# YzM1a0/MuDPT

Measured on AMD Instinct MI355X. Metric: images/sec fwd+bwd ViT-B/16 MuDPT, higher is better.
Workload: dtype bf16; 1 GPU; MuDPT ViT-B/16 fwd+bwd+SGD, batch 256/GPU, 11 class prompts, n_ctx 4, depth 12, synthetic 224x224 N(0,1) images, random-init frozen CLIP (BASELINE configs[1]); global_batch=256, parallelism=dp1

## Files before the change

mudpt_amd/csrc/gemm.hip:

```cpp
#include <type_traits>

#include "kernels.h"

namespace mudpt {

using gptr_t = const __attribute__((address_space(1))) void*;
using lptr_t = __attribute__((address_space(3))) void*;

template <typename T, int BM, int BN, int WM, int WN, int EPI, int NS = 2, int BK = 64>
__global__ __launch_bounds__(WM* WN * 64) void gemm_nt_kernel(GemmArgs p) {
    using elem = typename T::elem;
    using vec8 = typename T::vec8;
    constexpr int NW = WM * WN;
    static_assert(BK == 64 || BK == 128, "K-tile");
    constexpr int ROWB = BK * 2;
    constexpr int RPI = 1024 / ROWB;
    constexpr int CPR = ROWB / 16;
    constexpr int TM = BM / WM / 16;
    constexpr int TN = BN / WN / 16;
    constexpr int IA = BM / RPI / NW;
    constexpr int IB = BN / RPI / NW;
    constexpr int STAGE_BYTES = (BM + BN) * ROWB;
    static_assert(BM % (RPI * NW) == 0 && BN % (RPI * NW) == 0, "tile rows must split over the waves");

// ... 302 lines not shown
    ARG_CHECK(!a.gelu_q8 || ((epi == EPI_GELU && !a.out1_lo) || epi == EPI_GELU_BWD), "gemm: gelu_q8 belongs to the QuickGELU epilogues (1 without a split output, 3)");
    ARG_CHECK(a.lo_mode == LO_NONE || a.lo_mode == LO_F16 || a.lo_mode == LO_F8, "gemm: bad lo_mode %d", a.lo_mode);
    if (a.lo_mode != LO_NONE) ARG_CHECK(a.A_lo && (uintptr_t)a.A_lo % 16 == 0, "gemm: a split operand needs its low half (16-byte aligned)");
    if (a.lo_mode == LO_F8) {
        ARG_CHECK(dtype == DT_F16, "gemm: the e4m3 second pass exists for fp16 operands only");
        ARG_CHECK(a.B8 && (uintptr_t)a.B8 % 16 == 0 && a.K % 128 == 0, "gemm: the e4m3 second pass needs B8 and K %% 128 == 0 (K = %d)", a.K);
        ARG_CHECK(a.b8_scale > 0 && a.b8_scale < 255, "gemm: bad E8M0 weight scale %d", a.b8_scale);
    }
    if (epi == EPI_RESIDUAL || epi == EPI_GELU_BWD) ARG_CHECK(a.aux && a.ldaux >= a.N && a.ldaux % 4 == 0, "gemm: epilogue needs aux");
    if (epi == EPI_PATCH) ARG_CHECK(a.pos && a.patches > 0 && a.seq_len > a.patches && a.M % a.patches == 0, "gemm: bad patch epilogue args");
    GemmArgs b = a;
    if (variant & 0x100) b.flags |= 1;
    if (variant & 0x200) b.flags |= 2;
    b.flags |= ((variant >> 10) & 3) << 4;
    b.flags |= ((variant >> 12) & 0xff) << 8;
    if (gemm_uses_pp(epi, a, o.variant)) return launch_gemm_pp(dtype, epi, b, s, o);
    bool deep = false;
    if (const int S = split_k_slices(epi, a, o, deep); S > 1) {
        GemmArgs q = b;
        q.bias = nullptr; q.out0 = o.scratch; q.ldo0 = a.N; q.ksplit = a.K / S; q.split_stride = (size_t)a.M * a.N;
        if (dtype == DT_BF16) { if (int rc = deep ? launch_cfg<BF16, 64, 64, 2, 2, EPI_STORE_F32, 2, 128>(q, s) : launch_cfg<BF16, 64, 64, 2, 2, EPI_STORE_F32, 2>(q, s)) return rc; }
        else if (dtype == DT_F16) { if (int rc = deep ? launch_cfg<F16, 64, 64, 2, 2, EPI_STORE_F32, 2, 128>(q, s) : launch_cfg<F16, 64, 64, 2, 2, EPI_STORE_F32, 2>(q, s)) return rc; }
        else { set_error("gemm: unknown dtype %d", dtype); return MUDPT_ERR_ARG; }
        const unsigned grid = (unsigned)(((size_t)a.M * (a.N / 4) + 255) / 256);
        if (epi == EPI_STORE_F32) hipLaunchKernelGGL((splitk_reduce_kernel<BF16, true>), dim3(grid), dim3(256), 0, s, o.scratch, S, q.split_stride, a.M, a.N, a.bias, a.out0, a.ldo0);
        else if (dtype == DT_BF16) hipLaunchKernelGGL((splitk_reduce_kernel<BF16, false>), dim3(grid), dim3(256), 0, s, o.scratch, S, q.split_stride, a.M, a.N, a.bias, a.out0, a.ldo0);
        else hipLaunchKernelGGL((splitk_reduce_kernel<F16, false>), dim3(grid), dim3(256), 0, s, o.scratch, S, q.split_stride, a.M, a.N, a.bias, a.out0, a.ldo0);
        HIP_TRY(hipGetLastError());
        return MUDPT_OK;
    }
    if (dtype == DT_BF16) return launch_t<BF16>(epi, b, s, o.variant);
// ... 7 lines not shown
```

mudpt_amd/csrc/kernels.h:

```cpp
#pragma once
#include "common.h"

namespace mudpt {

enum Epilogue : int {
    EPI_STORE = 0,
    EPI_GELU = 1,
    EPI_RESIDUAL = 2,
    EPI_GELU_BWD = 3,
    EPI_PATCH = 4,
    EPI_STORE_F32 = 5
};

struct GemmArgs {
    const void* A = nullptr;
    const void* B = nullptr;
    int M = 0, N = 0, K = 0, lda = 0, ldb = 0;
    const float* bias = nullptr;
    void* out0 = nullptr; int ldo0 = 0;
    void* out1 = nullptr; int ldo1 = 0;
    void* out1_lo = nullptr;
    int out1_lo_mode = LO_F16;
    const void* A_lo = nullptr; int lo_mode = LO_NONE;
    const void* B8 = nullptr; int b8_scale = 127;
    const void* aux = nullptr; int ldaux = 0;
    bool gelu_q8 = false;
    int flags = 0;
    int patches = 0, seq_len = 0;
    const float* pos = nullptr;
    int ksplit = 0; size_t split_stride = 0;
};
struct GemmOpts {
    int variant = 0;
    hipEvent_t ev_start = nullptr, ev_stop = nullptr;
    float* scratch = nullptr; size_t scratch_elems = 0;
};
int launch_gemm(int dtype, int epi, const GemmArgs& a, hipStream_t s, const GemmOpts& o = GemmOpts());
bool gemm_uses_pp(int epi, const GemmArgs& a, int variant = 0);
int launch_gemm_pp(int dtype, int epi, const GemmArgs& a, hipStream_t s, const GemmOpts& o);

struct LnFwdArgs {
    const float* x = nullptr; int ldx = 0;
    const int* row_index = nullptr;
    const float* gamma = nullptr; const float* beta = nullptr;
    void* out = nullptr; int ldo = 0;
    void* out_lo = nullptr;
    int lo_mode = LO_F16;
    float* mean = nullptr; float* rstd = nullptr;
    int rows = 0, d = 0; bool out_f32 = false;
    const float* add = nullptr; int ldadd = 0;
    const void* add_lp = nullptr;
    float* xout = nullptr; int ldxout = 0;
    const float* ov_rows = nullptr; int ov_row0 = 0, ov_n = 0, ov_L = 1;
};
int launch_ln_fwd(int dtype, const LnFwdArgs& a, hipStream_t s, const LaunchProf* prof = nullptr);

struct LnBwdArgs {
    const void* dy = nullptr; int lddy = 0; bool dy_f32 = false;
    const float* x = nullptr; int ldx = 0;
    const int* row_index = nullptr;
    const float* mean = nullptr; const float* rstd = nullptr; const float* gamma = nullptr;
    const float* dres = nullptr; int lddres = 0;
    const void* dres_lp = nullptr;
    float* dx = nullptr; int lddx = 0;
    void* dx_lp = nullptr; int lddx_lp = 0;
    int rows = 0, d = 0;
    bool by_token = false;
    bool stats_by_token = false;
    float* side = nullptr; int side_row0 = 0, side_n = 0, side_L = 1; size_t side_ldb = 0;
};
int launch_ln_bwd(int dtype, const LnBwdArgs& a, hipStream_t s, const LaunchProf* prof = nullptr);

struct AttnArgs {
    const void* qkv = nullptr;
    void* out = nullptr;
    void* out_lo = nullptr;
    int lo_mode = LO_F16;
    int ld_out = 0;
    float* lse = nullptr;
    const void* dout = nullptr;
    void* dqkv = nullptr;
// ... 73 lines not shown
```

mudpt_amd/csrc/layernorm.hip:

```cpp
#include "kernels.h"

namespace mudpt {

constexpr int LN_MAXV = 4;

template <typename T, bool OUT_F32>
__global__ __launch_bounds__(256) void ln_fwd_kernel(LnFwdArgs p) {
    using elem = typename T::elem;
    const int lane = threadIdx.x & 63;
    const int r = blockIdx.x * 4 + (threadIdx.x >> 6);
    if (r >= p.rows) return;
    const size_t xr = p.row_index ? (size_t)p.row_index[r] : (size_t)r;
    const f32x4* x = (const f32x4*)(p.x + xr * p.ldx);
    const int d4 = p.d >> 2;
    f32x4 v[LN_MAXV];
    float s = 0.f;
    const f32x4* ov = nullptr;
    if (p.ov_rows) {
        const int pos = r % p.ov_L - p.ov_row0;
        if (pos >= 0 && pos < p.ov_n) ov = (const f32x4*)(p.ov_rows + (size_t)pos * p.d);
    }
    const f32x4* add = (p.add && !ov) ? (const f32x4*)(p.add + xr * p.ldadd) : nullptr;
    const typename T::vec4* add_lp = (p.add_lp && !ov) ? (const typename T::vec4*)((const elem*)p.add_lp + xr * p.ldadd) : nullptr;
#pragma unroll
    for (int k = 0; k < LN_MAXV; ++k) {
// ... 42 lines not shown
                    if (p.lo_mode == LO_F8) ((uint32_t*)((char*)p.out_lo + (size_t)r * p.ldo * 2))[i] = pack_lo8(rem[0], rem[1], rem[2], rem[3]);
                    else ((typename T::vec4*)((elem*)p.out_lo + (size_t)r * p.ldo))[i] = lo;
                } else {
                    typename T::vec4 o = {(elem)y[0], (elem)y[1], (elem)y[2], (elem)y[3]};
                    ((typename T::vec4*)((elem*)p.out + (size_t)r * p.ldo))[i] = o;
                }
            }
        }
    }
}

template <typename T, bool DY_F32>
__global__ __launch_bounds__(256) void ln_bwd_kernel(LnBwdArgs p) {
    using elem = typename T::elem;
    const int lane = threadIdx.x & 63;
    const int r = blockIdx.x * 4 + (threadIdx.x >> 6);
    if (r >= p.rows) return;
    const size_t t = p.row_index ? (size_t)p.row_index[r] : (size_t)r;
    const f32x4* x = (const f32x4*)(p.x + t * p.ldx);
    const int d4 = p.d >> 2;
    const size_t sr = p.by_token ? t : (size_t)r;
    const size_t st = (p.by_token || p.stats_by_token) ? t : (size_t)r;
    const float mean = p.mean[st], rstd = p.rstd[st];
    f32x4* side_row = nullptr;
    if (p.side) {
        const int pos = (int)(t % (size_t)p.side_L) - p.side_row0;
        if (pos >= 0 && pos < p.side_n) side_row = (f32x4*)(p.side + (t / (size_t)p.side_L) * p.side_ldb + (size_t)pos * p.d);
    }
    f32x4 xh[LN_MAXV], g[LN_MAXV];
    typename T::vec4 rv[LN_MAXV];
    float s1 = 0.f, s2 = 0.f;
// ... 36 lines not shown
            }
            if (side_row) { side_row[i] = dx; dx = f32x4{0.f, 0.f, 0.f, 0.f}; }
            if (p.dx) ((f32x4*)(p.dx + t * p.lddx))[i] = dx;
            if (p.dx_lp) {
                typename T::vec4 o = {(elem)dx[0], (elem)dx[1], (elem)dx[2], (elem)dx[3]};
                ((typename T::vec4*)((elem*)p.dx_lp + t * p.lddx_lp))[i] = o;
            }
        }
    }
}

int launch_ln_fwd(int dtype, const LnFwdArgs& a, hipStream_t s, const LaunchProf* prof) {
    ARG_CHECK(a.x && a.gamma && a.beta && a.out, "ln_fwd: null operand");
    ARG_CHECK(a.rows > 0 && a.d > 0 && a.d % 4 == 0 && a.d <= 256 * LN_MAXV, "ln_fwd: bad shape rows=%d d=%d", a.rows, a.d);
    ARG_CHECK(a.ldx % 4 == 0 && a.ldo % 4 == 0 && a.ldx >= a.d && a.ldo >= a.d, "ln_fwd: bad strides %d/%d", a.ldx, a.ldo);
    const dim3 grid((a.rows + 3) / 4), block(256);
    if (dtype == DT_BF16) {
        if (a.out_f32) MUDPT_LAUNCH((ln_fwd_kernel<BF16, true>), grid, block, 0, s, prof, a);
        else MUDPT_LAUNCH((ln_fwd_kernel<BF16, false>), grid, block, 0, s, prof, a);
    } else if (dtype == DT_F16) {
        if (a.out_f32) MUDPT_LAUNCH((ln_fwd_kernel<F16, true>), grid, block, 0, s, prof, a);
        else MUDPT_LAUNCH((ln_fwd_kernel<F16, false>), grid, block, 0, s, prof, a);
    } else {
        set_error("ln_fwd: unknown dtype %d", dtype);
        return MUDPT_ERR_ARG;
    }
    HIP_TRY(hipGetLastError());
    return MUDPT_OK;
}

int launch_ln_bwd(int dtype, const LnBwdArgs& a, hipStream_t s, const LaunchProf* prof) {
    ARG_CHECK(a.dy && a.x && a.mean && a.rstd && a.gamma && (a.dx || a.dx_lp), "ln_bwd: null operand");
    ARG_CHECK(!(a.dres && a.dres_lp), "ln_bwd: dres and dres_lp are exclusive");
    ARG_CHECK(!a.side || (!a.row_index && a.side_L > 0 && a.side_n > 0), "ln_bwd: the fused splice backward needs the identity row map");
    ARG_CHECK(a.rows > 0 && a.d > 0 && a.d % 4 == 0 && a.d <= 256 * LN_MAXV, "ln_bwd: bad shape rows=%d d=%d", a.rows, a.d);
    ARG_CHECK(a.ldx % 4 == 0 && a.lddy % 4 == 0 && a.lddx % 4 == 0, "ln_bwd: strides must be multiples of 4");
    const dim3 grid((a.rows + 3) / 4), block(256);
    if (dtype == DT_BF16) {
        if (a.dy_f32) MUDPT_LAUNCH((ln_bwd_kernel<BF16, true>), grid, block, 0, s, prof, a);
        else MUDPT_LAUNCH((ln_bwd_kernel<BF16, false>), grid, block, 0, s, prof, a);
    } else if (dtype == DT_F16) {
        if (a.dy_f32) MUDPT_LAUNCH((ln_bwd_kernel<F16, true>), grid, block, 0, s, prof, a);
        else MUDPT_LAUNCH((ln_bwd_kernel<F16, false>), grid, block, 0, s, prof, a);
    } else {
        set_error("ln_bwd: unknown dtype %d", dtype);
        return MUDPT_ERR_ARG;
    }
    HIP_TRY(hipGetLastError());
    return MUDPT_OK;
}

}
// ... 1 lines not shown
```

mudpt_amd/csrc/model.cpp:

```cpp
#include <dlfcn.h>
#include <stdarg.h>
#include <stdio.h>
#include <string.h>

#include <algorithm>
#include <cmath>
#include <string>
#include <vector>

#include "../../include/mudpt.h"
#include "kernels.h"

namespace mudpt {

static thread_local char g_err[1024] = "";
void set_error(const char* fmt, ...) {
    va_list ap;
    va_start(ap, fmt);
    vsnprintf(g_err, sizeof(g_err), fmt, ap);
    va_end(ap);
}
const char* get_error() { return g_err; }

static inline uint16_t f32_to_bf16(float f) {
// ... 53 lines not shown
    bool may_split = false;
    int sites = 0x1f;
    void *h_lo = nullptr, *g_lo = nullptr, *attn_lo = nullptr;
    void *h_sel_lo = nullptr, *g_sel_lo = nullptr, *attn_sel_lo = nullptr;
    int prompt_row0 = 0;
    std::vector<BlockW> w;
    std::vector<BlockAct> a;
    void *h = nullptr, *g = nullptr;
    bool exact_attn = false;
    float* qkv32 = nullptr;
    float* dx = nullptr; void* dx_lp = nullptr;
    void *dattn = nullptr, *dqkv = nullptr;
    float* delta = nullptr;
    float* upd = nullptr;
    const int* tail_rows = nullptr;
    float *xin_sel = nullptr, *xmid_sel = nullptr, *xout_sel = nullptr;
    void *attn_sel = nullptr, *h_sel = nullptr, *u_sel = nullptr, *g_sel = nullptr, *dattn_sel = nullptr;
    float* dsel = nullptr; void* dsel_lp = nullptr;
    void *q_sel = nullptr, *dq_sel = nullptr, *dqx_sel = nullptr;
    float* lse_sel = nullptr;
    const int* head_rows = nullptr;
    int head_n = 0;
    void *hd_dqkv = nullptr, *hd_h = nullptr;
    std::vector<void*> act_allocs;
    struct Seg { int row0 = 0, seq0 = 0, nseq = 0, L = 0; size_t lse0 = 0; };
    std::vector<Seg> segs;
    int rows = 0;
    const int* tail_local = nullptr;
};

// ... 63 lines not shown
    bool attn_fused_w1 = false;
    bool split_k = true;
    bool fwd_split_k = true;
    bool train_fwd = false;
    static constexpr size_t kFwdSplitTiles = 320;
    static constexpr size_t kScratchElems = (size_t)4 << 20;
    float *gemm_scratch = nullptr, *gemm_scratch2 = nullptr;
    bool attn_window = true;
    bool last_single = true;
    bool attn_two_kernels = false;
    int cocoop_chunk = 0;
    int txt_chunk = 1;
    bool any_weight_set = false;
    hipStream_t s2 = nullptr;
    hipEvent_t ev_fork = nullptr, ev_join = nullptr, ev_fork_b = nullptr, ev_join_b = nullptr;
    bool prof = false;
    int prof_mask = 0;
    int prof_stride = 1;
    long pp_seen = 0;
    std::vector<hipEvent_t> ev;
    size_t ev_used = 0;
    struct ProfRec { int cls; double work; };
    std::vector<ProfRec> ev_rec;
    double exec_flop = 0;
};
enum ProfClass : int { PC_GEMM = 0, PC_LN_FWD = 1, PC_LN_BWD = 2, PC_ATTN_FWD = 3, PC_ATTN_BWD = 4, PC_COUNT = 5 };

static int prof_next(mudpt_model* m, int cls, double work, LaunchProf* out) {
    *out = LaunchProf();
    if (!m->prof || !(m->prof_mask & (1 << cls))) return MUDPT_OK;
    if (m->ev_used + 2 > m->ev.size()) {
        for (int i = 0; i < 512; ++i) {
            hipEvent_t e;
            HIP_TRY(hipEventCreate(&e));
            m->ev.push_back(e);
        }
    }
    out->start = m->ev[m->ev_used];
    out->stop = m->ev[m->ev_used + 1];
    m->ev_used += 2;
    m->ev_rec.push_back({cls, work});
    return MUDPT_OK;
}

static int gemm_call(mudpt_model* m, int epi, const GemmArgs& a, hipStream_t s, bool bwd = false, bool fwd_split = false) {
    GemmOpts o;
    o.variant = m->gemm_variant;
    const bool fwd_small = fwd_split && m->fwd_split_k && m->train_fwd && (size_t)((a.M + 63) / 64) * ((a.N + 63) / 64) <= mudpt_model::kFwdSplitTiles;
    if (m->split_k && (bwd || fwd_small)) {
        o.scratch = s == m->s2 ? m->gemm_scratch2 : m->gemm_scratch;
        o.scratch_elems = mudpt_model::kScratchElems;
    }
    if (m->prof) m->exec_flop += 2.0 * a.M * a.N * a.K;
    if (!m->prof || !gemm_uses_pp(epi, a, o.variant)) return launch_gemm(m->dtype, epi, a, s, o);
    if (m->prof_stride > 1 && (m->pp_seen++ % m->prof_stride) != 0) return launch_gemm(m->dtype, epi, a, s, o);
    LaunchProf lp;
    if (int rc = prof_next(m, PC_GEMM, 2.0 * a.M * a.N * a.K, &lp)) return rc;
    o.ev_start = lp.start;
    o.ev_stop = lp.stop;
    return launch_gemm(m->dtype, epi, a, s, o);
}

static bool prof_big(const mudpt_model* m, const Tower& t, int rows) { return m->prof && &t == &m->vis && rows >= 4096; }
static int ln_fwd_call(mudpt_model* m, const Tower& t, const LnFwdArgs& a, hipStream_t s) {
    if (!prof_big(m, t, a.rows)) return launch_ln_fwd(m->dtype, a, s);
    const double per_elem = 4.0 + (a.add ? 4.0 : 0.0) + (a.add_lp ? 2.0 : 0.0) + (a.xout ? 4.0 : 0.0) + (a.out_f32 ? 4.0 : 2.0) + (a.out_lo ? 2.0 : 0.0);
    LaunchProf lp;
    if (int rc = prof_next(m, PC_LN_FWD, per_elem * a.rows * a.d, &lp)) return rc;
    return launch_ln_fwd(m->dtype, a, s, &lp);
}
static int ln_bwd_call(mudpt_model* m, const Tower& t, const LnBwdArgs& a, hipStream_t s) {
    if (!prof_big(m, t, a.rows)) return launch_ln_bwd(m->dtype, a, s);
    const double per_elem = (a.dy_f32 ? 4.0 : 2.0) + 4.0 + (a.dres ? 4.0 : 0.0) + (a.dres_lp ? 2.0 : 0.0) + (a.dx ? 4.0 : 0.0) + (a.dx_lp ? 2.0 : 0.0);
    LaunchProf lp;
    if (int rc = prof_next(m, PC_LN_BWD, per_elem * a.rows * a.d, &lp)) return rc;
    return launch_ln_bwd(m->dtype, a, s, &lp);
}
static int attn_call(mudpt_model* m, const Tower& t, const AttnArgs& a0, bool bwd, hipStream_t s) {
    AttnArgs a = a0;
    a.two_kernels = m->attn_two_kernels;
    a.fused_w1 = m->attn_fused_w1;
    const double prod = 2.0 * a.L * (double)a.L * 64.0 * a.H * a.B * (a.causal ? 0.5 : 1.0);
    const bool exact_fwd = !bwd && a.qkv32;
    if (m->prof && !a.sel_rows && !exact_fwd) m->exec_flop += (bwd ? 7.0 : 2.0) * prod;
    if (exact_fwd) return launch_attn_fwd_exact(a, s);
    if (!prof_big(m, t, a.B * a.L) || a.sel_rows) return bwd ? launch_attn_bwd(m->dtype, a, s) : launch_attn_fwd(m->dtype, a, s);
    const double tok = (double)a.B * a.L * a.H * 128.0;
    LaunchProf lp;
    if (int rc = prof_next(m, bwd ? PC_ATTN_BWD : PC_ATTN_FWD, bwd ? 8.0 * tok : (4.0 + (a.out_lo ? 1.0 : 0.0)) * tok, &lp)) return rc;
    return bwd ? launch_attn_bwd(m->dtype, a, s, &lp) : launch_attn_fwd(m->dtype, a, s, &lp);
}

// ... 171 lines not shown
        ALLOC(m->vis_deep, dn * dv * 4); ALLOC(m->txt_deep, dn * dt * 4);
        ALLOC(m->vsplice, (size_t)B * dn * dv * 4);
        ALLOC(m->d_vis_deep, dn * dv * 4); ALLOC(m->d_txt_deep, dn * dt * 4); ALLOC(m->d_vprompt0, (size_t)n * dv * 4);
        ALLOC(m->img_f, (size_t)B * e * 4); ALLOC(m->txt_f, (size_t)TS * e * 4); ALLOC(m->img_n, (size_t)B * e * 4); ALLOC(m->txt_n, (size_t)TS * e * 4);
        ALLOC(m->img_inv, B * 4); ALLOC(m->txt_inv, TS * 4);
        ALLOC(m->logits, (size_t)B * C * 4); ALLOC(m->dlogits, (size_t)B * C * 4); ALLOC(m->row_loss, B * 4);
        ALLOC(m->dimg, (size_t)B * e * 4); ALLOC(m->dtxt, (size_t)TS * e * 4); ALLOC(m->loss, 16);
        if (cocoop) {
            m->hid = e / 16;
            ALLOC(m->mn_hid, (size_t)B * m->hid * 4); ALLOC(m->mn_dhid, (size_t)B * m->hid * 4);
            ALLOC(m->mn_bias, (size_t)B * dt * 4); ALLOC(m->mn_dbias, (size_t)B * dt * 4);
        }
        ALLOC(m->gemm_scratch, mudpt_model::kScratchElems * 4); ALLOC(m->gemm_scratch2, mudpt_model::kScratchElems * 4);
        HIP_TRY(hipStreamCreateWithFlags(&m->s2, hipStreamNonBlocking));
        for (hipEvent_t* e : {&m->ev_fork, &m->ev_join, &m->ev_fork_b, &m->ev_join_b}) HIP_TRY(hipEventCreateWithFlags(e, hipEventDisableTiming));
        std::vector<int> cr(B), pr((size_t)B * n);
        for (int b = 0; b < B; ++b) {
            cr[b] = b * Lv;
            for (int i = 0; i < n; ++i) pr[(size_t)b * n + i] = b * Lv + (Lv - n) + i;
        }
        HIP_TRY(hipMemcpy(m->cls_rows, cr.data(), cr.size() * 4, hipMemcpyHostToDevice));
        m->vis.tail_rows = m->cls_rows;
        m->vis.head_rows = cocoop ? nullptr : m->vprompt_rows;
        ALLOC(m->tprompt_rows, (size_t)TS * n * 4);
        m->txt.head_rows = m->tprompt_rows;
        m->txt.tail_rows = m->eot_rows;
        HIP_TRY(hipMemcpy(m->vprompt_rows, pr.data(), pr.size() * 4, hipMemcpyHostToDevice));
        return MUDPT_OK;
    };
    if (int r = body()) return fail(r);
// ... 11 lines not shown
                          "visual.ln_pre.bias", "visual.ln_post.weight", "visual.ln_post.bias", "visual.proj", "positional_embedding",
                          "ln_final.weight", "ln_final.bias", "text_projection", "logit_scale"})
        m->missing.push_back(k);
    expect_block_keys(m, "visual.transformer", c->v_layers);
    expect_block_keys(m, "transformer", c->t_layers);
    *out = m;
    return MUDPT_OK;
}

extern "C" int mudpt_destroy(mudpt_model* m) {
    if (!m) return MUDPT_OK;
    for (void* p : m->allocs) (void)hipFree(p);
    for (Tower* t : {&m->vis, &m->txt})
        for (void* p : t->act_allocs) (void)hipFree(p);
    for (hipEvent_t e : m->ev) (void)hipEventDestroy(e);
    for (hipEvent_t e : {m->ev_fork, m->ev_join, m->ev_fork_b, m->ev_join_b})
        if (e) (void)hipEventDestroy(e);
    if (m->s2) (void)hipStreamDestroy(m->s2);
    delete m;
    return MUDPT_OK;
}

static int upload_f32(float* dst, const float* src, size_t n) {
    HIP_TRY(hipMemcpy(dst, src, n * 4, hipMemcpyHostToDevice));
    return MUDPT_OK;
}
static int upload_lp(int dtype, void* dst, void* dst_t, const float* src, size_t rows, size_t cols) {
    std::vector<uint16_t> tmp(rows * cols);
    auto cv = [&](float f) { return dtype == DT_BF16 ? f32_to_bf16(f) : f32_to_f16(f); };
    for (size_t i = 0; i < rows * cols; ++i) tmp[i] = cv(src[i]);
    HIP_TRY(hipMemcpy(dst, tmp.data(), tmp.size() * 2, hipMemcpyHostToDevice));
    if (dst_t) {
        for (size_t r = 0; r < rows; ++r)
// ... 293 lines not shown
    if (m_fc != LO_NONE) { l2.out_lo = t.h_sel_lo; l2.lo_mode = m_fc; }
    TRY(launch_ln_fwd(dt, l2, s));
    GemmArgs f; f.A = t.h_sel; f.lda = d; f.B = w.w_fc; f.ldb = d; f.M = S; f.N = 4 * d; f.K = d; f.bias = w.b_fc;
    split_operand(f, m_fc, t.h_sel_lo, w.w_fc8, w.s_fc8);
    f.out0 = t.u_sel; f.ldo0 = 4 * d; f.out1 = t.g_sel; f.ldo1 = 4 * d;
    f.gelu_q8 = m->gelu_q8 && t.split == LO_NONE;
    if (m_proj != LO_NONE) { f.out1_lo = t.g_sel_lo; f.out1_lo_mode = m_proj; }
    TRY(gemm_call(m, EPI_GELU, f, s));
    GemmArgs p; p.A = t.g_sel; p.lda = 4 * d; p.B = w.w_proj; p.ldb = 4 * d; p.M = S; p.N = d; p.K = 4 * d; p.bias = w.b_proj;
    split_operand(p, m_proj, t.g_sel_lo, w.w_proj8, w.s_proj8);
    p.out0 = t.xout_sel; p.ldo0 = d; p.aux = t.xmid_sel; p.ldaux = d;
    TRY(gemm_call(m, EPI_RESIDUAL, p, s));
    return MUDPT_OK;
}

static int block_fwd(mudpt_model* m, Tower& t, int i, int nseq, const float* splice, hipStream_t s) {
    const int M = tower_rows(t, nseq), d = t.d, dt = m->dtype, n = m->cfg.n_ctx;
    const std::vector<Tower::Seg> segs = tower_segs(t, nseq);
    const bool lp = m->lp_upd;
    BlockW& w = t.w[i];
    BlockAct& a = t.a[i];
    const size_t esz = 2;
    const int m_qkv = site_mode(t, SITE_QKV, d), m_out = site_mode(t, SITE_OUT, d), m_fc = site_mode(t, SITE_FC, d), m_proj = site_mode(t, SITE_PROJ, 4 * d);
    LnFwdArgs l1; l1.x = a.x_in; l1.ldx = d; l1.gamma = w.ln1_g; l1.beta = w.ln1_b; l1.out = t.h; l1.ldo = d; l1.mean = a.mean1; l1.rstd = a.rstd1; l1.rows = M; l1.d = d;
    if (m_qkv != LO_NONE) { l1.out_lo = t.h_lo; l1.lo_mode = m_qkv; }
    if (i > 0) {
        l1.x = t.a[i - 1].x_mid; l1.ldadd = d; l1.xout = a.x_in; l1.ldxout = d;
        if (lp) l1.add_lp = t.upd; else l1.add = t.upd;
        if (splice) { l1.ov_rows = splice; l1.ov_row0 = t.prompt_row0; l1.ov_n = n; l1.ov_L = t.L; }
    }
    if (splice && i > 0 && segs.size() > 1) {
        for (const Tower::Seg& g : segs) {
            LnFwdArgs b = l1;
            const size_t r0 = (size_t)g.row0;
            b.x = l1.x + r0 * l1.ldx; b.xout = l1.xout + r0 * l1.ldxout;
            if (l1.add) b.add = l1.add + r0 * l1.ldadd;
            if (l1.add_lp) b.add_lp = (const char*)l1.add_lp + r0 * l1.ldadd * esz;
            b.out = (char*)l1.out + r0 * l1.ldo * esz;
            if (l1.out_lo) b.out_lo = (char*)l1.out_lo + r0 * l1.ldo * esz;
            b.mean = l1.mean + r0; b.rstd = l1.rstd + r0; b.rows = g.nseq * g.L; b.ov_L = g.L;
            TRY(ln_fwd_call(m, t, b, s));
        }
    } else {
        TRY(ln_fwd_call(m, t, l1, s));
    }
    if (i + 1 == t.layers && m->last_single && !t.exact_attn && t.tail_rows) {
// ... 19 lines not shown
    GemmArgs q; q.A = t.h; q.lda = d; q.B = w.w_in; q.ldb = d; q.M = M; q.N = 3 * d; q.K = d; q.bias = w.b_in; q.out0 = a.qkv; q.ldo0 = 3 * d;
    split_operand(q, m_qkv, t.h_lo, w.w_in8, w.s_in8);
    if (t.exact_attn) q.out0 = t.qkv32;
    TRY(gemm_call(m, t.exact_attn ? EPI_STORE_F32 : EPI_STORE, q, s));
    for (const Tower::Seg& g : segs) {
        AttnArgs at; at.qkv = (const char*)a.qkv + (size_t)g.row0 * 3 * d * esz; at.out = (char*)a.attn + (size_t)g.row0 * d * esz; at.lse = a.lse + g.lse0;
        at.B = g.nseq; at.L = g.L; at.H = t.heads; at.causal = t.causal;
        if (m_out != LO_NONE) { at.out_lo = (char*)t.attn_lo + (size_t)g.row0 * d * esz; at.lo_mode = m_out; }
        if (t.exact_attn) { at.qkv32 = t.qkv32 + (size_t)g.row0 * 3 * d; at.qkv_lp = (char*)a.qkv + (size_t)g.row0 * 3 * d * esz; }
        TRY(attn_call(m, t, at, false, s));
    }
    if (i + 1 == t.layers) return block_fwd_tail(m, t, nseq, s);
    GemmArgs o; o.A = a.attn; o.lda = d; o.B = w.w_out; o.ldb = d; o.M = M; o.N = d; o.K = d; o.bias = w.b_out; o.out0 = t.upd; o.ldo0 = d;
    split_operand(o, m_out, t.attn_lo, w.w_out8, w.s_out8);
    const bool fs = !t.causal && t.split == LO_NONE;
    TRY(gemm_call(m, lp ? EPI_STORE : EPI_STORE_F32, o, s, false, fs));
    LnFwdArgs l2; l2.x = a.x_in; l2.ldx = d; if (lp) l2.add_lp = t.upd; else l2.add = t.upd; l2.ldadd = d; l2.xout = a.x_mid; l2.ldxout = d; l2.gamma = w.ln2_g; l2.beta = w.ln2_b; l2.out = t.h; l2.ldo = d;
    if (m_fc != LO_NONE) { l2.out_lo = t.h_lo; l2.lo_mode = m_fc; }
    l2.mean = a.mean2; l2.rstd = a.rstd2; l2.rows = M; l2.d = d;
    TRY(ln_fwd_call(m, t, l2, s));
    GemmArgs f; f.A = t.h; f.lda = d; f.B = w.w_fc; f.ldb = d; f.M = M; f.N = 4 * d; f.K = d; f.bias = w.b_fc; f.out0 = a.u; f.ldo0 = 4 * d;
    split_operand(f, m_fc, t.h_lo, w.w_fc8, w.s_fc8);
    f.out1 = t.g; f.ldo1 = 4 * d;
    f.gelu_q8 = m->gelu_q8 && t.split == LO_NONE;
    if (m_proj != LO_NONE) { f.out1_lo = t.g_lo; f.out1_lo_mode = m_proj; }
    TRY(gemm_call(m, EPI_GELU, f, s));
    GemmArgs p; p.A = t.g; p.lda = 4 * d; p.B = w.w_proj; p.ldb = 4 * d; p.M = M; p.N = d; p.K = 4 * d; p.bias = w.b_proj; p.out0 = t.upd; p.ldo0 = d;
    split_operand(p, m_proj, t.g_lo, w.w_proj8, w.s_proj8);
    TRY(gemm_call(m, lp ? EPI_STORE : EPI_STORE_F32, p, s, false, fs));
    return MUDPT_OK;
}

static int block_bwd_tail(mudpt_model* m, Tower& t, int nseq, hipStream_t s) {
    const int i = t.layers - 1, M = tower_rows(t, nseq), S = nseq, d = t.d, dt = m->dtype;
    const std::vector<Tower::Seg> segs = tower_segs(t, nseq);
    const size_t esz = 2;
    BlockW& w = t.w[i];
    BlockAct& a = t.a[i];
    GemmArgs g1; g1.A = t.dsel_lp; g1.lda = d; g1.B = w.w_proj_t; g1.ldb = d; g1.M = S; g1.N = 4 * d; g1.K = d; g1.out0 = t.g_sel; g1.ldo0 = 4 * d; g1.aux = t.u_sel; g1.ldaux = 4 * d;
    g1.gelu_q8 = m->gelu_q8 && t.split == LO_NONE;
    TRY(gemm_call(m, EPI_GELU_BWD, g1, s, !t.causal));
    GemmArgs g2; g2.A = t.g_sel; g2.lda = 4 * d; g2.B = w.w_fc_t; g2.ldb = 4 * d; g2.M = S; g2.N = d; g2.K = 4 * d; g2.out0 = t.h_sel; g2.ldo0 = d;
    TRY(gemm_call(m, EPI_STORE, g2, s, !t.causal));
// ... 40 lines not shown
    LnBwdArgs b1; b1.dy = t.h; b1.lddy = d; b1.x = a.x_in; b1.ldx = d; b1.mean = a.mean1; b1.rstd = a.rstd1; b1.gamma = w.ln1_g; b1.lddres = d;
    if (m->lp_grad) b1.dres_lp = t.dx_lp; else { b1.dres = t.dx; b1.dx = t.dx; }
    b1.lddx = d; b1.dx_lp = t.dx_lp; b1.lddx_lp = d; b1.rows = M; b1.d = d;
    TRY(ln_bwd_call(m, t, b1, s));
    return MUDPT_OK;
}

static int block_bwd(mudpt_model* m, Tower& t, int i, int nseq, hipStream_t s, float* side = nullptr, size_t side_ldb = 0) {
    const int M = tower_rows(t, nseq), d = t.d, dt = m->dtype;
    BlockW& w = t.w[i];
    BlockAct& a = t.a[i];
    GemmArgs g1; g1.A = t.dx_lp; g1.lda = d; g1.B = w.w_proj_t; g1.ldb = d; g1.M = M; g1.N = 4 * d; g1.K = d; g1.out0 = t.g; g1.ldo0 = 4 * d; g1.aux = a.u; g1.ldaux = 4 * d;
    g1.gelu_q8 = m->gelu_q8 && t.split == LO_NONE;
    TRY(gemm_call(m, EPI_GELU_BWD, g1, s, !t.causal));
    GemmArgs g2; g2.A = t.g; g2.lda = 4 * d; g2.B = w.w_fc_t; g2.ldb = 4 * d; g2.M = M; g2.N = d; g2.K = 4 * d; g2.out0 = t.h; g2.ldo0 = d;
    TRY(gemm_call(m, EPI_STORE, g2, s, !t.causal));
    LnBwdArgs b2; b2.dy = t.h; b2.lddy = d; b2.x = a.x_mid; b2.ldx = d; b2.mean = a.mean2; b2.rstd = a.rstd2; b2.gamma = w.ln2_g; b2.lddres = d;
    if (m->lp_grad) b2.dres_lp = t.dx_lp; else { b2.dres = t.dx; b2.dx = t.dx; }
    b2.lddx = d; b2.dx_lp = t.dx_lp; b2.lddx_lp = d; b2.rows = M; b2.d = d;
    TRY(ln_bwd_call(m, t, b2, s));
    GemmArgs g3; g3.A = t.dx_lp; g3.lda = d; g3.B = w.w_out_t; g3.ldb = d; g3.M = M; g3.N = d; g3.K = d; g3.out0 = t.dattn; g3.ldo0 = d;
    TRY(gemm_call(m, EPI_STORE, g3, s, !t.causal));
    for (const Tower::Seg& g : tower_segs(t, nseq)) {
        const size_t esz = 2;
        AttnArgs at; at.qkv = (const char*)a.qkv + (size_t)g.row0 * 3 * d * esz; at.out = (char*)a.attn + (size_t)g.row0 * d * esz; at.lse = a.lse + g.lse0;
        at.dout = (const char*)t.dattn + (size_t)g.row0 * d * esz; at.dqkv = (char*)t.dqkv + (size_t)g.row0 * 3 * d * esz; at.delta = t.delta + g.lse0;
        at.B = g.nseq; at.L = g.L; at.H = t.heads; at.causal = t.causal;
        if (i == 0 && t.head_rows && t.layers > 1 && m->attn_window) { at.win_row0 = t.prompt_row0; at.win_n = t.head_n; }
        TRY(attn_call(m, t, at, true, s));
    }
    if (i == 0 && t.head_rows && t.layers > 1) {
        const int R = nseq * t.head_n;
        TRY(launch_gather_rows(t.dqkv, (size_t)3 * d * 2, t.head_rows, t.hd_dqkv, (size_t)3 * d * 2, R, 3 * d * 2, s));
        GemmArgs g4; g4.A = t.hd_dqkv; g4.lda = 3 * d; g4.B = w.w_in_t; g4.ldb = 3 * d; g4.M = R; g4.N = d; g4.K = 3 * d; g4.out0 = t.hd_h; g4.ldo0 = d;
        TRY(gemm_call(m, EPI_STORE, g4, s, !t.causal));
        LnBwdArgs b1; b1.dy = t.hd_h; b1.lddy = d; b1.x = a.x_in; b1.ldx = d; b1.row_index = t.head_rows; b1.stats_by_token = true;
        b1.mean = a.mean1; b1.rstd = a.rstd1; b1.gamma = w.ln1_g; b1.lddres = d;
        if (m->lp_grad) b1.dres_lp = t.dx_lp; else { b1.dres = t.dx; b1.dx = t.dx; }
        b1.lddx = d; b1.dx_lp = t.dx_lp; b1.lddx_lp = d; b1.rows = R; b1.d = d;
        TRY(launch_ln_bwd(dt, b1, s));
        return MUDPT_OK;
    }
    GemmArgs g4; g4.A = t.dqkv; g4.lda = 3 * d; g4.B = w.w_in_t; g4.ldb = 3 * d; g4.M = M; g4.N = d; g4.K = 3 * d; g4.out0 = t.h; g4.ldo0 = d;
    TRY(gemm_call(m, EPI_STORE, g4, s, !t.causal));
    LnBwdArgs b1; b1.dy = t.h; b1.lddy = d; b1.x = a.x_in; b1.ldx = d; b1.mean = a.mean1; b1.rstd = a.rstd1; b1.gamma = w.ln1_g; b1.lddres = d;
    if (m->lp_grad) b1.dres_lp = t.dx_lp; else { b1.dres = t.dx; b1.dx = t.dx; }
    b1.lddx = d; b1.dx_lp = t.dx_lp; b1.lddx_lp = d; b1.rows = M; b1.d = d;
    if (side) { b1.side = side; b1.side_row0 = t.prompt_row0; b1.side_n = m->cfg.n_ctx; b1.side_L = t.L; b1.side_ldb = side_ldb; }
    TRY(ln_bwd_call(m, t, b1, s));
    return MUDPT_OK;
}

static int vision_forward(mudpt_model* m, const float* images, int B, hipStream_t s) {
    const mudpt_config& c = m->cfg;
    const int dv = c.v_width, e = c.embed_dim, n = c.n_ctx, D1 = c.depth - 1;
    const int P = (c.image_size / c.patch) * (c.image_size / c.patch), Lv = m->vis.L, K0 = (3 * c.patch * c.patch + 63) / 64 * 64;
    float* Pm = m->params;
    const int m_patch = site_mode(m->vis, SITE_PATCH, K0);
    if (m_patch != LO_NONE) TRY(launch_patchify_split(m->dtype, images, m->patches, m->patches_lo, m_patch, B, c.image_size, c.patch, K0, s));
    else TRY(launch_patchify(m->dtype, images, m->patches, B, c.image_size, c.patch, K0, s));
    GemmArgs pe; pe.A = m->patches; pe.lda = K0; pe.B = m->conv_w; pe.ldb = K0; pe.M = B * P; pe.N = dv; pe.K = K0; pe.out0 = m->xpre; pe.ldo0 = dv;
    split_operand(pe, m_patch, m->patches_lo, m->conv_w8, m->conv_s8);
    pe.patches = P; pe.seq_len = Lv; pe.pos = m->vpos;
    TRY(gemm_call(m, EPI_PATCH, pe, s));
    TRY(launch_set_rows(m->xpre, B, Lv, dv, 0, 1, m->cls, m->vpos, s));
    if (!m->cocoop) TRY(launch_set_rows(m->xpre, B, Lv, dv, Lv - n, n, Pm + m->off[P_VCTX], m->shared, s));
    LnFwdArgs lp; lp.x = m->xpre; lp.ldx = dv; lp.gamma = m->ln_pre_g; lp.beta = m->ln_pre_b; lp.out = m->vis.a[0].x_in; lp.ldo = dv; lp.out_f32 = true;
    lp.mean = m->pre_mean; lp.rstd = m->pre_rstd; lp.rows = B * Lv; lp.d = dv;
    TRY(launch_ln_fwd(m->dtype, lp, s));
    for (int i = 0; i < m->vis.layers; ++i) {
        TRY(block_fwd(m, m->vis, i, B, (i >= 1 && i - 1 < D1) ? m->vis_deep + (size_t)(i - 1) * n * dv : nullptr, s));
    }
    LnFwdArgs lq; lq.x = m->vis.xout_sel; lq.ldx = dv; lq.gamma = m->ln_post_g; lq.beta = m->ln_post_b; lq.out = m->f_ln; lq.ldo = dv;
    lq.out_f32 = true; lq.mean = m->post_mean; lq.rstd = m->post_rstd; lq.rows = B; lq.d = dv;
    TRY(launch_ln_fwd(m->dtype, lq, s));
    TRY(launch_sgemm(false, false, B, e, dv, 1.f, m->f_ln, dv, m->vproj, e, 0.f, m->img_f, e, nullptr, s));
    return MUDPT_OK;
}

static int cocoop_text_chunk(mudpt_model* m, int i0, int nb, hipStream_t s) {
    const mudpt_config& c = m->cfg;
    const int dt = c.t_width, e = c.embed_dim, n = c.n_ctx, C = c.n_cls, Lt = m->txt.L, TS = nb * C;
    const size_t r0 = (size_t)i0 * C;
    TRY(launch_cocoop_prompts(m->txt.a[0].x_in, m->emb_pos, m->params + m->off[Q_CTX], m->mn_bias + (size_t)i0 * dt, m->tpos, nb, C, Lt, dt, n, s));
    for (int i = 0; i < m->txt.layers; ++i) TRY(block_fwd(m, m->txt, i, TS, nullptr, s));
    LnFwdArgs lf; lf.x = m->txt.xout_sel; lf.ldx = dt; lf.gamma = m->ln_fin_g; lf.beta = m->ln_fin_b; lf.out = m->t_ln + r0 * dt; lf.ldo = dt;
// ... 405 lines not shown
    m->loss_scale = loss_scale;
    return MUDPT_OK;
}

extern "C" int mudpt_model_set(mudpt_model* m, const char* name, int32_t value) {
    ARG_CHECK(m && name, "model_set: null argument");
    if (!strcmp(name, "gemm_variant")) { m->gemm_variant = value; return MUDPT_OK; }
    if (!strcmp(name, "lp_grad")) { m->lp_grad = value != 0; if (m->dtype == MUDPT_BF16) m->lp_upd = value != 0; return MUDPT_OK; }
    if (!strcmp(name, "lp_upd")) { m->lp_upd = value != 0; return MUDPT_OK; }
    if (!strcmp(name, "gelu_q8")) { m->gelu_q8 = value != 0; return MUDPT_OK; }
    if (!strcmp(name, "txt_trim")) { m->txt_trim = value != 0; m->prompts_set = false; return MUDPT_OK; }
    if (!strcmp(name, "attn_two_kernels")) { m->attn_two_kernels = value != 0; return MUDPT_OK; }
    if (!strcmp(name, "fwd_split_k")) { m->fwd_split_k = value != 0; return MUDPT_OK; }
    if (!strcmp(name, "attn_fused_w1")) { m->attn_fused_w1 = value != 0; return MUDPT_OK; }
    if (!strcmp(name, "split_k")) { m->split_k = value != 0; return MUDPT_OK; }
    if (!strcmp(name, "attn_window")) { m->attn_window = value != 0; return MUDPT_OK; }
    if (!strcmp(name, "last_single")) { m->last_single = value != 0; return MUDPT_OK; }
    if (!strcmp(name, "txt_bucket_cost")) { m->txt_bucket_cost = value > 0 ? value : 0; m->prompts_set = false; return MUDPT_OK; }
    if (!strcmp(name, "txt_buckets")) { m->txt_buckets = value > 1 ? value : 1; m->prompts_set = false; return MUDPT_OK; }
    if (!strcmp(name, "prof_stride")) { m->prof_stride = value > 1 ? value : 1; return MUDPT_OK; }
    if (!strcmp(name, "cocoop_chunk")) { m->cocoop_chunk = value; m->prompts_set = false; return MUDPT_OK; }
    for (Tower* t : {&m->vis, &m->txt}) {
        const char* pre = t == &m->vis ? "vis_" : "txt_";
        if (strncmp(name, pre, 4)) continue;
        const char* k = name + 4;
        if (!strcmp(k, "lo") || (t == &m->txt && !strcmp(k, "split"))) {
            if (value != LO_NONE && !t->may_split) { set_error("model_set: %s needs a mode whose %s tower keeps low halves (dtype fp32%s)", name, t == &m->vis ? "vision" : "text", t == &m->txt ? " or fp16" : ""); return MUDPT_ERR_STATE; }
            ARG_CHECK(value == LO_NONE || value == LO_F16 || (value == LO_F8 && !t->w.empty() && t->w[0].w_in8), "model_set: %s = %d is not available for this tower", name, value);
            t->split = value;
            m->text_valid = false;
// ... 198 lines not shown
```

Measured before the change: 11020 images/s.

## Split vision GEMMs into row panels and overlap LayerNorm on a third stream

For vision-tower GEMMs followed by a LayerNorm (out-proj→LN2, fc2→next LN1, and the backward dX GEMMs→LN backward), the GEMM is split into a full-wave panel part and a tail. The LayerNorm for the first rows runs on a new stream while the tail GEMM runs, which fills the partial last wave of CUs. The next block's LN1 is hoisted into the previous block's fc2 step. This adds a row0 offset to the LN kernels, a force_pp flag, extra events and stream syncs, and more launches per block.

```diff
diff --git a/mudpt_amd/csrc/gemm.hip b/mudpt_amd/csrc/gemm.hip
--- a/mudpt_amd/csrc/gemm.hip
+++ b/mudpt_amd/csrc/gemm.hip
@@ -340,7 +340,7 @@
     if (variant & 0x200) b.flags |= 2;
     b.flags |= ((variant >> 10) & 3) << 4;
     b.flags |= ((variant >> 12) & 0xff) << 8;
-    if (gemm_uses_pp(epi, a, o.variant)) return launch_gemm_pp(dtype, epi, b, s, o);
+    if (o.force_pp || gemm_uses_pp(epi, a, o.variant)) return launch_gemm_pp(dtype, epi, b, s, o);
     bool deep = false;
     if (const int S = split_k_slices(epi, a, o, deep); S > 1) {
         GemmArgs q = b;
diff --git a/mudpt_amd/csrc/kernels.h b/mudpt_amd/csrc/kernels.h
--- a/mudpt_amd/csrc/kernels.h
+++ b/mudpt_amd/csrc/kernels.h
@@ -32,6 +32,7 @@
 };
 struct GemmOpts {
     int variant = 0;
+    bool force_pp = false;
     hipEvent_t ev_start = nullptr, ev_stop = nullptr;
     float* scratch = nullptr; size_t scratch_elems = 0;
 };
@@ -48,6 +49,7 @@
     int lo_mode = LO_F16;
     float* mean = nullptr; float* rstd = nullptr;
     int rows = 0, d = 0; bool out_f32 = false;
+    int row0 = 0;
     const float* add = nullptr; int ldadd = 0;
     const void* add_lp = nullptr;
     float* xout = nullptr; int ldxout = 0;
@@ -65,6 +67,7 @@
     float* dx = nullptr; int lddx = 0;
     void* dx_lp = nullptr; int lddx_lp = 0;
     int rows = 0, d = 0;
+    int row0 = 0;
     bool by_token = false;
     bool stats_by_token = false;
     float* side = nullptr; int side_row0 = 0, side_n = 0, side_L = 1; size_t side_ldb = 0;
diff --git a/mudpt_amd/csrc/layernorm.hip b/mudpt_amd/csrc/layernorm.hip
--- a/mudpt_amd/csrc/layernorm.hip
+++ b/mudpt_amd/csrc/layernorm.hip
@@ -8,7 +8,7 @@
 __global__ __launch_bounds__(256) void ln_fwd_kernel(LnFwdArgs p) {
     using elem = typename T::elem;
     const int lane = threadIdx.x & 63;
-    const int r = blockIdx.x * 4 + (threadIdx.x >> 6);
+    const int r = p.row0 + blockIdx.x * 4 + (threadIdx.x >> 6);
     if (r >= p.rows) return;
     const size_t xr = p.row_index ? (size_t)p.row_index[r] : (size_t)r;
     const f32x4* x = (const f32x4*)(p.x + xr * p.ldx);
@@ -81,7 +81,7 @@
 __global__ __launch_bounds__(256) void ln_bwd_kernel(LnBwdArgs p) {
     using elem = typename T::elem;
     const int lane = threadIdx.x & 63;
-    const int r = blockIdx.x * 4 + (threadIdx.x >> 6);
+    const int r = p.row0 + blockIdx.x * 4 + (threadIdx.x >> 6);
     if (r >= p.rows) return;
     const size_t t = p.row_index ? (size_t)p.row_index[r] : (size_t)r;
     const f32x4* x = (const f32x4*)(p.x + t * p.ldx);
@@ -148,7 +148,8 @@
     ARG_CHECK(a.x && a.gamma && a.beta && a.out, "ln_fwd: null operand");
     ARG_CHECK(a.rows > 0 && a.d > 0 && a.d % 4 == 0 && a.d <= 256 * LN_MAXV, "ln_fwd: bad shape rows=%d d=%d", a.rows, a.d);
     ARG_CHECK(a.ldx % 4 == 0 && a.ldo % 4 == 0 && a.ldx >= a.d && a.ldo >= a.d, "ln_fwd: bad strides %d/%d", a.ldx, a.ldo);
-    const dim3 grid((a.rows + 3) / 4), block(256);
+    ARG_CHECK(a.row0 >= 0 && a.row0 < a.rows, "ln_fwd: bad first row %d of %d", a.row0, a.rows);
+    const dim3 grid((a.rows - a.row0 + 3) / 4), block(256);
     if (dtype == DT_BF16) {
         if (a.out_f32) MUDPT_LAUNCH((ln_fwd_kernel<BF16, true>), grid, block, 0, s, prof, a);
         else MUDPT_LAUNCH((ln_fwd_kernel<BF16, false>), grid, block, 0, s, prof, a);
@@ -169,7 +170,8 @@
     ARG_CHECK(!a.side || (!a.row_index && a.side_L > 0 && a.side_n > 0), "ln_bwd: the fused splice backward needs the identity row map");
     ARG_CHECK(a.rows > 0 && a.d > 0 && a.d % 4 == 0 && a.d <= 256 * LN_MAXV, "ln_bwd: bad shape rows=%d d=%d", a.rows, a.d);
     ARG_CHECK(a.ldx % 4 == 0 && a.lddy % 4 == 0 && a.lddx % 4 == 0, "ln_bwd: strides must be multiples of 4");
-    const dim3 grid((a.rows + 3) / 4), block(256);
+    ARG_CHECK(a.row0 >= 0 && a.row0 < a.rows, "ln_bwd: bad first row %d of %d", a.row0, a.rows);
+    const dim3 grid((a.rows - a.row0 + 3) / 4), block(256);
     if (dtype == DT_BF16) {
         if (a.dy_f32) MUDPT_LAUNCH((ln_bwd_kernel<BF16, true>), grid, block, 0, s, prof, a);
         else MUDPT_LAUNCH((ln_bwd_kernel<BF16, false>), grid, block, 0, s, prof, a);
diff --git a/mudpt_amd/csrc/model.cpp b/mudpt_amd/csrc/model.cpp
--- a/mudpt_amd/csrc/model.cpp
+++ b/mudpt_amd/csrc/model.cpp
@@ -91,6 +91,7 @@
     float* delta = nullptr;
     float* upd = nullptr;
     const int* tail_rows = nullptr;
+    int ln1_done = -1;
     float *xin_sel = nullptr, *xmid_sel = nullptr, *xout_sel = nullptr;
     void *attn_sel = nullptr, *h_sel = nullptr, *u_sel = nullptr, *g_sel = nullptr, *dattn_sel = nullptr;
     float* dsel = nullptr; void* dsel_lp = nullptr;
@@ -184,6 +185,10 @@
     bool any_weight_set = false;
     hipStream_t s2 = nullptr;
     hipEvent_t ev_fork = nullptr, ev_join = nullptr, ev_fork_b = nullptr, ev_join_b = nullptr;
+    int ln_overlap = 2;
+    hipStream_t s3 = nullptr;
+    hipEvent_t ev_ln_a = nullptr, ev_ln_b = nullptr;
+    int ncu = 0;
     bool prof = false;
     int prof_mask = 0;
     int prof_stride = 1;
@@ -213,16 +218,17 @@
     return MUDPT_OK;
 }
 
-static int gemm_call(mudpt_model* m, int epi, const GemmArgs& a, hipStream_t s, bool bwd = false, bool fwd_split = false) {
+static int gemm_call(mudpt_model* m, int epi, const GemmArgs& a, hipStream_t s, bool bwd = false, bool fwd_split = false, bool force_pp = false) {
     GemmOpts o;
     o.variant = m->gemm_variant;
+    o.force_pp = force_pp;
     const bool fwd_small = fwd_split && m->fwd_split_k && m->train_fwd && (size_t)((a.M + 63) / 64) * ((a.N + 63) / 64) <= mudpt_model::kFwdSplitTiles;
     if (m->split_k && (bwd || fwd_small)) {
         o.scratch = s == m->s2 ? m->gemm_scratch2 : m->gemm_scratch;
         o.scratch_elems = mudpt_model::kScratchElems;
     }
     if (m->prof) m->exec_flop += 2.0 * a.M * a.N * a.K;
-    if (!m->prof || !gemm_uses_pp(epi, a, o.variant)) return launch_gemm(m->dtype, epi, a, s, o);
+    if (!m->prof || !(force_pp || gemm_uses_pp(epi, a, o.variant))) return launch_gemm(m->dtype, epi, a, s, o);
     if (m->prof_stride > 1 && (m->pp_seen++ % m->prof_stride) != 0) return launch_gemm(m->dtype, epi, a, s, o);
     LaunchProf lp;
     if (int rc = prof_next(m, PC_GEMM, 2.0 * a.M * a.N * a.K, &lp)) return rc;
@@ -246,6 +252,41 @@
     if (int rc = prof_next(m, PC_LN_BWD, per_elem * a.rows * a.d, &lp)) return rc;
     return launch_ln_bwd(m->dtype, a, s, &lp);
 }
+template <typename LnArgs>
+static int gemm_then_ln(mudpt_model* m, const Tower& t, int epi, const GemmArgs& a, const LnArgs& l, hipStream_t s, bool bwd, bool fwd_split,
+                        int (*ln)(mudpt_model*, const Tower&, const LnArgs&, hipStream_t)) {
+    int R = 0;
+    if (m->ln_overlap && m->s3 && m->ncu > 0 && &t == &m->vis && s != m->s2 && m->gemm_variant == 0 && l.row0 == 0 && l.rows == a.M && !l.row_index &&
+        gemm_uses_pp(epi, a, 0)) {
+        const int ntn = (a.N + 255) / 256, ntm = (a.M + 255) / 256;
+        const int panels = (ntm * ntn / m->ncu) * m->ncu / ntn;
+        if (panels > 0 && panels < ntm) R = panels * 256;
+    }
+    if (!R) {
+        if (int rc = gemm_call(m, epi, a, s, bwd, fwd_split)) return rc;
+        return ln(m, t, l, s);
+    }
+    GemmArgs g1 = a, g2 = a;
+    g1.M = R;
+    g2.M = a.M - R;
+    g2.A = (const char*)a.A + (size_t)R * a.lda * 2;
+    if (a.A_lo) g2.A_lo = (const char*)a.A_lo + (size_t)R * a.lda * 2;
+    g2.out0 = (char*)a.out0 + (size_t)R * a.ldo0 * (epi == EPI_STORE_F32 ? 4 : 2);
+    if (m->ln_overlap == 2) g2.flags |= 2;
+    LnArgs l1 = l, l2 = l;
+    l1.rows = R;
+    l2.row0 = R;
+    if (int rc = gemm_call(m, epi, g1, s, bwd, fwd_split)) return rc;
+    HIP_TRY(hipEventRecord(m->ev_ln_a, s));
+    if (int rc = gemm_call(m, epi, g2, s, bwd, fwd_split, true)) return rc;
+    HIP_TRY(hipStreamWaitEvent(m->s3, m->ev_ln_a, 0));
+    if (int rc = ln(m, t, l1, m->s3)) return rc;
+    HIP_TRY(hipEventRecord(m->ev_ln_b, m->s3));
+    if (int rc = ln(m, t, l2, s)) return rc;
+    HIP_TRY(hipStreamWaitEvent(s, m->ev_ln_b, 0));
+    return MUDPT_OK;
+}
+
 static int attn_call(mudpt_model* m, const Tower& t, const AttnArgs& a0, bool bwd, hipStream_t s) {
     AttnArgs a = a0;
     a.two_kernels = m->attn_two_kernels;
@@ -447,6 +488,9 @@
         ALLOC(m->gemm_scratch, mudpt_model::kScratchElems * 4); ALLOC(m->gemm_scratch2, mudpt_model::kScratchElems * 4);
         HIP_TRY(hipStreamCreateWithFlags(&m->s2, hipStreamNonBlocking));
         for (hipEvent_t* e : {&m->ev_fork, &m->ev_join, &m->ev_fork_b, &m->ev_join_b}) HIP_TRY(hipEventCreateWithFlags(e, hipEventDisableTiming));
+        HIP_TRY(hipStreamCreateWithFlags(&m->s3, hipStreamNonBlocking));
+        for (hipEvent_t* e : {&m->ev_ln_a, &m->ev_ln_b}) HIP_TRY(hipEventCreateWithFlags(e, hipEventDisableTiming));
+        HIP_TRY(hipDeviceGetAttribute(&m->ncu, hipDeviceAttributeMultiprocessorCount, current_device()));
         std::vector<int> cr(B), pr((size_t)B * n);
         for (int b = 0; b < B; ++b) {
             cr[b] = b * Lv;
@@ -488,9 +532,10 @@
     for (Tower* t : {&m->vis, &m->txt})
         for (void* p : t->act_allocs) (void)hipFree(p);
     for (hipEvent_t e : m->ev) (void)hipEventDestroy(e);
-    for (hipEvent_t e : {m->ev_fork, m->ev_join, m->ev_fork_b, m->ev_join_b})
+    for (hipEvent_t e : {m->ev_fork, m->ev_join, m->ev_fork_b, m->ev_join_b, m->ev_ln_a, m->ev_ln_b})
         if (e) (void)hipEventDestroy(e);
     if (m->s2) (void)hipStreamDestroy(m->s2);
+    if (m->s3) (void)hipStreamDestroy(m->s3);
     delete m;
     return MUDPT_OK;
 }
@@ -814,22 +859,33 @@
     return MUDPT_OK;
 }
 
-static int block_fwd(mudpt_model* m, Tower& t, int i, int nseq, const float* splice, hipStream_t s) {
-    const int M = tower_rows(t, nseq), d = t.d, dt = m->dtype, n = m->cfg.n_ctx;
+static LnFwdArgs ln1_args(const mudpt_model* m, Tower& t, int i, int M, const float* splice) {
+    const int d = t.d, n = m->cfg.n_ctx, m_qkv = site_mode(t, SITE_QKV, d);
+    BlockW& w = t.w[i];
+    BlockAct& a = t.a[i];
+    LnFwdArgs l1; l1.x = a.x_in; l1.ldx = d; l1.gamma = w.ln1_g; l1.beta = w.ln1_b; l1.out = t.h; l1.ldo = d; l1.mean = a.mean1; l1.rstd = a.rstd1; l1.rows = M; l1.d = d;
+    if (m_qkv != LO_NONE) { l1.out_lo = t.h_lo; l1.lo_mode = m_qkv; }
+    if (i > 0) {
+        l1.x = t.a[i - 1].x_mid; l1.ldadd = d; l1.xout = a.x_in; l1.ldxout = d;
+        if (m->lp_upd) l1.add_lp = t.upd; else l1.add = t.upd;
+        if (splice) { l1.ov_rows = splice; l1.ov_row0 = t.prompt_row0; l1.ov_n = n; l1.ov_L = t.L; }
+    }
+    return l1;
+}
+
+static int block_fwd(mudpt_model* m, Tower& t, int i, int nseq, const float* splice, hipStream_t s, const float* next_splice = nullptr) {
+    const int M = tower_rows(t, nseq), d = t.d, dt = m->dtype;
     const std::vector<Tower::Seg> segs = tower_segs(t, nseq);
     const bool lp = m->lp_upd;
     BlockW& w = t.w[i];
     BlockAct& a = t.a[i];
     const size_t esz = 2;
     const int m_qkv = site_mode(t, SITE_QKV, d), m_out = site_mode(t, SITE_OUT, d), m_fc = site_mode(t, SITE_FC, d), m_proj = site_mode(t, SITE_PROJ, 4 * d);
-    LnFwdArgs l1; l1.x = a.x_in; l1.ldx = d; l1.gamma = w.ln1_g; l1.beta = w.ln1_b; l1.out = t.h; l1.ldo = d; l1.mean = a.mean1; l1.rstd = a.rstd1; l1.rows = M; l1.d = d;
-    if (m_qkv != LO_NONE) { l1.out_lo = t.h_lo; l1.lo_mode = m_qkv; }
-    if (i > 0) {
-        l1.x = t.a[i - 1].x_mid; l1.ldadd = d; l1.xout = a.x_in; l1.ldxout = d;
-        if (lp) l1.add_lp = t.upd; else l1.add = t.upd;
-        if (splice) { l1.ov_rows = splice; l1.ov_row0 = t.prompt_row0; l1.ov_n = n; l1.ov_L = t.L; }
-    }
-    if (splice && i > 0 && segs.size() > 1) {
+    const LnFwdArgs l1 = ln1_args(m, t, i, M, splice);
+    const bool l1_done = i > 0 && t.ln1_done == i;
+    t.ln1_done = -1;
+    if (l1_done) {
+    } else if (splice && i > 0 && segs.size() > 1) {
         for (const Tower::Seg& g : segs) {
             LnFwdArgs b = l1;
             const size_t r0 = (size_t)g.row0;
@@ -879,11 +935,10 @@
     GemmArgs o; o.A = a.attn; o.lda = d; o.B = w.w_out; o.ldb = d; o.M = M; o.N = d; o.K = d; o.bias = w.b_out; o.out0 = t.upd; o.ldo0 = d;
     split_operand(o, m_out, t.attn_lo, w.w_out8, w.s_out8);
     const bool fs = !t.causal && t.split == LO_NONE;
-    TRY(gemm_call(m, lp ? EPI_STORE : EPI_STORE_F32, o, s, false, fs));
     LnFwdArgs l2; l2.x = a.x_in; l2.ldx = d; if (lp) l2.add_lp = t.upd; else l2.add = t.upd; l2.ldadd = d; l2.xout = a.x_mid; l2.ldxout = d; l2.gamma = w.ln2_g; l2.beta = w.ln2_b; l2.out = t.h; l2.ldo = d;
     if (m_fc != LO_NONE) { l2.out_lo = t.h_lo; l2.lo_mode = m_fc; }
     l2.mean = a.mean2; l2.rstd = a.rstd2; l2.rows = M; l2.d = d;
-    TRY(ln_fwd_call(m, t, l2, s));
+    TRY(gemm_then_ln(m, t, lp ? EPI_STORE : EPI_STORE_F32, o, l2, s, false, fs, ln_fwd_call));
     GemmArgs f; f.A = t.h; f.lda = d; f.B = w.w_fc; f.ldb = d; f.M = M; f.N = 4 * d; f.K = d; f.bias = w.b_fc; f.out0 = a.u; f.ldo0 = 4 * d;
     split_operand(f, m_fc, t.h_lo, w.w_fc8, w.s_fc8);
     f.out1 = t.g; f.ldo1 = 4 * d;
@@ -892,6 +947,11 @@
     TRY(gemm_call(m, EPI_GELU, f, s));
     GemmArgs p; p.A = t.g; p.lda = 4 * d; p.B = w.w_proj; p.ldb = 4 * d; p.M = M; p.N = d; p.K = 4 * d; p.bias = w.b_proj; p.out0 = t.upd; p.ldo0 = d;
     split_operand(p, m_proj, t.g_lo, w.w_proj8, w.s_proj8);
+    if (&t == &m->vis && !(next_splice && segs.size() > 1)) {
+        TRY(gemm_then_ln(m, t, lp ? EPI_STORE : EPI_STORE_F32, p, ln1_args(m, t, i + 1, M, next_splice), s, false, fs, ln_fwd_call));
+        t.ln1_done = i + 1;
+        return MUDPT_OK;
+    }
     TRY(gemm_call(m, lp ? EPI_STORE : EPI_STORE_F32, p, s, false, fs));
     return MUDPT_OK;
 }
@@ -962,11 +1022,10 @@
     g1.gelu_q8 = m->gelu_q8 && t.split == LO_NONE;
     TRY(gemm_call(m, EPI_GELU_BWD, g1, s, !t.causal));
     GemmArgs g2; g2.A = t.g; g2.lda = 4 * d; g2.B = w.w_fc_t; g2.ldb = 4 * d; g2.M = M; g2.N = d; g2.K = 4 * d; g2.out0 = t.h; g2.ldo0 = d;
-    TRY(gemm_call(m, EPI_STORE, g2, s, !t.causal));
     LnBwdArgs b2; b2.dy = t.h; b2.lddy = d; b2.x = a.x_mid; b2.ldx = d; b2.mean = a.mean2; b2.rstd = a.rstd2; b2.gamma = w.ln2_g; b2.lddres = d;
     if (m->lp_grad) b2.dres_lp = t.dx_lp; else { b2.dres = t.dx; b2.dx = t.dx; }
     b2.lddx = d; b2.dx_lp = t.dx_lp; b2.lddx_lp = d; b2.rows = M; b2.d = d;
-    TRY(ln_bwd_call(m, t, b2, s));
+    TRY(gemm_then_ln(m, t, EPI_STORE, g2, b2, s, !t.causal, false, ln_bwd_call));
     GemmArgs g3; g3.A = t.dx_lp; g3.lda = d; g3.B = w.w_out_t; g3.ldb = d; g3.M = M; g3.N = d; g3.K = d; g3.out0 = t.dattn; g3.ldo0 = d;
     TRY(gemm_call(m, EPI_STORE, g3, s, !t.causal));
     for (const Tower::Seg& g : tower_segs(t, nseq)) {
@@ -990,12 +1049,11 @@
         return MUDPT_OK;
     }
     GemmArgs g4; g4.A = t.dqkv; g4.lda = 3 * d; g4.B = w.w_in_t; g4.ldb = 3 * d; g4.M = M; g4.N = d; g4.K = 3 * d; g4.out0 = t.h; g4.ldo0 = d;
-    TRY(gemm_call(m, EPI_STORE, g4, s, !t.causal));
     LnBwdArgs b1; b1.dy = t.h; b1.lddy = d; b1.x = a.x_in; b1.ldx = d; b1.mean = a.mean1; b1.rstd = a.rstd1; b1.gamma = w.ln1_g; b1.lddres = d;
     if (m->lp_grad) b1.dres_lp = t.dx_lp; else { b1.dres = t.dx; b1.dx = t.dx; }
     b1.lddx = d; b1.dx_lp = t.dx_lp; b1.lddx_lp = d; b1.rows = M; b1.d = d;
     if (side) { b1.side = side; b1.side_row0 = t.prompt_row0; b1.side_n = m->cfg.n_ctx; b1.side_L = t.L; b1.side_ldb = side_ldb; }
-    TRY(ln_bwd_call(m, t, b1, s));
+    TRY(gemm_then_ln(m, t, EPI_STORE, g4, b1, s, !t.causal, false, ln_bwd_call));
     return MUDPT_OK;
 }
 
@@ -1017,7 +1075,8 @@
     lp.mean = m->pre_mean; lp.rstd = m->pre_rstd; lp.rows = B * Lv; lp.d = dv;
     TRY(launch_ln_fwd(m->dtype, lp, s));
     for (int i = 0; i < m->vis.layers; ++i) {
-        TRY(block_fwd(m, m->vis, i, B, (i >= 1 && i - 1 < D1) ? m->vis_deep + (size_t)(i - 1) * n * dv : nullptr, s));
+        auto splice = [&](int j) -> const float* { return (j >= 1 && j - 1 < D1) ? m->vis_deep + (size_t)(j - 1) * n * dv : nullptr; };
+        TRY(block_fwd(m, m->vis, i, B, splice(i), s, splice(i + 1)));
     }
     LnFwdArgs lq; lq.x = m->vis.xout_sel; lq.ldx = dv; lq.gamma = m->ln_post_g; lq.beta = m->ln_post_b; lq.out = m->f_ln; lq.ldo = dv;
     lq.out_f32 = true; lq.mean = m->post_mean; lq.rstd = m->post_rstd; lq.rows = B; lq.d = dv;
@@ -1453,6 +1512,7 @@
     if (!strcmp(name, "fwd_split_k")) { m->fwd_split_k = value != 0; return MUDPT_OK; }
     if (!strcmp(name, "attn_fused_w1")) { m->attn_fused_w1 = value != 0; return MUDPT_OK; }
     if (!strcmp(name, "split_k")) { m->split_k = value != 0; return MUDPT_OK; }
+    if (!strcmp(name, "ln_overlap")) { m->ln_overlap = value >= 0 && value <= 2 ? value : 0; return MUDPT_OK; }
     if (!strcmp(name, "attn_window")) { m->attn_window = value != 0; return MUDPT_OK; }
     if (!strcmp(name, "last_single")) { m->last_single = value != 0; return MUDPT_OK; }
     if (!strcmp(name, "txt_bucket_cost")) { m->txt_bucket_cost = value > 0 ? value : 0; m->prompts_set = false; return MUDPT_OK; }
```

Result: no change. 11130 images/s, median of 6 (+1.0%).
